# Marcus-Forte/moptimizer_0

Measured on NVIDIA B200. Metric: point2point_linearized_residuals_per_sec, higher is better.
Workload: dtype f32

## Files before the change

### moptimizer_0_b200/csrc/mopt_capi.cu

```cuda
#include <dlfcn.h>

#include <cmath>
#include <atomic>
#include <chrono>
#include <cstdlib>
#include <cstring>
#include <mutex>

#include "mopt_internal.h"

using namespace mopt;

namespace {
thread_local std::string g_last_error;
}
namespace mopt {
void set_last_error(const std::string& msg) { g_last_error = msg; }
int store_upload_async(mopt_store* st, int group, const void* host, int host_dtype, int64_t host_stride, int64_t first,
                       int64_t count);
}

namespace {
struct NcclApi {
  typedef struct ncclComm* comm_t;
// ... 167 lines not shown
  }
  return MOPT_OK;
}

void fill_cost(const mopt_problem* p, CostDev* c) {
  std::memset(c, 0, sizeof(*c));
  c->model = p->model; c->variant = p->variant; c->P = p->num_parameters; c->O = p->num_outputs;
  c->jacobian = p->jacobian; c->loss = p->loss; c->has_cov = p->has_covariance ? 1 : 0;
  c->compute_dtype = p->compute_dtype; c->loss_param = p->loss_param;
  c->manifold = p->manifold;
  c->rot_offset = (p->model == MOPT_MODEL_POINT2POINT || p->model == MOPT_MODEL_PINHOLE ||
                   p->model == MOPT_MODEL_PINHOLE_DISTORT) ? 3 : -1;
  if (p->model >= MOPT_MODEL_USER_BASE) c->rot_offset = user_model_rot_offset(p->model);
  c->so3_guard = ((p->flags & MOPT_FLAG_REFERENCE_FLOAT_GUARD) && p->compute_dtype == MOPT_F32) ? kSo3GuardF32 : kSo3GuardF64;
  const int O = p->num_outputs;
  for (int i = 0; i < O * O; ++i) c->cov[i] = p->has_covariance ? p->covariance[i] : ((i % (O + 1) == 0) ? 1.0 : 0.0);
  std::memcpy(c->consts, p->consts, sizeof(c->consts));
}

int stage_cost(mopt_ctx* ctx, int i, const mopt_problem* p) {
  CostDev c;
  fill_cost(p, &c);
  if (ctx->cached_valid[i] && std::memcmp(&c, &ctx->cached_cost[i], sizeof(c)) == 0) return MOPT_OK;
  MOPT_CUDA_TRY(cudaStreamSynchronize(ctx->stream));
  ctx->h_slot->cost = c;
  MOPT_CUDA_TRY(cudaMemcpyAsync(&ctx->d_slots[i].cost, &ctx->h_slot->cost, sizeof(CostDev), cudaMemcpyHostToDevice, ctx->stream));
  MOPT_CUDA_TRY(cudaStreamSynchronize(ctx->stream));
  ctx->cached_cost[i] = c;
  ctx->cached_valid[i] = true;
  return MOPT_OK;
}

PassArgs make_args(mopt_ctx* ctx, const mopt_store* st, int slot, int accumulate, int mode_override) {
  PassArgs a;
  std::memset(&a, 0, sizeof(a));
  for (int s = 0; s < kMaxStreams; ++s) a.streams.p[s] = st->streams[s];
  a.n = st->n;
  a.pb = &ctx->d_slots[slot].pb;
  a.cost = &ctx->d_slots[slot].cost;
  a.partials = ctx->d_partials;
  a.ticket = ctx->d_ticket;
  a.out = ctx->d_trial;
  a.accumulate = accumulate;
  a.mode_ptr = &ctx->d_lm->pass_mode;
  a.mode_override = mode_override;
  a.masked = st->may_have_invalid ? 1 : 0;
// ... 15 lines not shown
}

int launch_pass(mopt_ctx* ctx, const mopt_store* st, const mopt_problem* p, int slot, int accumulate, int mode_override,
                bool push, const XArg* fused_x = nullptr) {
  PassArgs a = make_args(ctx, st, slot, accumulate, mode_override);
  if (fused_x) {
    a.fused_setup = 1;
    a.x = *fused_x;
  }
  if (push && ctx->world > 1 && ctx->peers_open && ctx->exchange_enabled) {
    for (int r = 0; r < ctx->world; ++r) a.peer.base[r] = ctx->peer_base[r];
    a.peer.world = ctx->world;
    a.peer.rank = ctx->rank;
    a.peer.push = 1;
    a.peer.fused = ctx->fused_consumer ? 1 : 0;
    a.peer.err = ctx->d_xerr;
    a.peer.err_dev = ctx->d_xerr_dev;
    a.peer.seq = ++ctx->xseq;
  }
  PassLaunch L{ctx->stream, ctx->num_sms, ctx->ctas_per_sm, ctx->threads};
  L.affine_fd = (p->compute_dtype == MOPT_F32) ? !(p->flags & MOPT_FLAG_GENERIC_KERNEL)
                                               : ((p->flags & MOPT_FLAG_STABLE_FD) && !(p->flags & MOPT_FLAG_GENERIC_KERNEL));
  L.identity_cov = !p->has_covariance;
  if (p->model >= MOPT_MODEL_USER_BASE)
    return launch_user(L, ctx->device, p->model, p->jacobian != MOPT_JAC_ANALYTICAL, st->dtype, p->compute_dtype, a);
  if (p->model == MOPT_MODEL_POINT2POINT && p->jacobian == MOPT_JAC_ANALYTICAL)
    return launch_p2p_moment(L, st->dtype, p->compute_dtype, p->loss,
                             p->variant == MOPT_P2P_EXACT || p->variant == MOPT_P2P_LEFT, a);
  if (p->model == MOPT_MODEL_POINT2POINT && !(p->flags & MOPT_FLAG_GENERIC_KERNEL) &&
      !(st->dtype == MOPT_F64 && p->compute_dtype == MOPT_F32))
    return launch_p2p_moment(L, st->dtype, p->compute_dtype, p->loss, false, a);
  if (p->model == MOPT_MODEL_PINHOLE_DISTORT) return launch_wide(L, p->model, st->dtype, p->compute_dtype, a);
  return launch_dense(L, p->model, p->jacobian != MOPT_JAC_ANALYTICAL, st->dtype, p->compute_dtype, a);
}

int allreduce_trial(mopt_ctx* ctx, int P, int mode_override) {
  if (ctx->world <= 1 || !ctx->exchange_enabled) return MOPT_OK;
  if (ctx->peers_open) {
    if (ctx->fused_consumer) return MOPT_OK;
    peer_reduce_kernel<<<1, 64, 0, ctx->stream>>>(ctx->d_xbuf, ctx->world, ctx->xseq, ctx->d_trial, packed_size(P),
                                                  &ctx->d_lm->pass_mode, mode_override, ctx->d_xerr, ctx->d_xerr_dev);
    MOPT_CUDA_TRY(cudaGetLastError());
    return MOPT_OK;
  }
  if (!ctx->nccl_comm) {
    set_last_error("sharded context has neither a NCCL communicator nor an open peer exchange");
// ... 19 lines not shown

int check_exchange_alive(const mopt_ctx* ctx) {
  if (ctx->h_xerr && *reinterpret_cast<volatile int*>(ctx->h_xerr)) {
    set_last_error("an earlier peer exchange on this context timed out (a rank died); destroy the context");
    return MOPT_ERR_COMM;
  }
  return MOPT_OK;
}

int enqueue_pass(mopt_ctx* ctx, mopt_store* st, const mopt_problem* p, const double* x, int mode) {
  MOPT_TRY(check_exchange_alive(ctx));
  MOPT_CUDA_TRY(cudaSetDevice(ctx->device));
  MOPT_TRY(stage_cost(ctx, 0, p));
  const int P = p->num_parameters;
  XArg xa;
  std::memset(&xa, 0, sizeof(xa));
  if (P > 0) {
    MOPT_REQUIRE(x != nullptr, "null parameter vector");
    for (int i = 0; i < P; ++i) xa.v[i] = x[i];
  }
  if (can_fuse_setup(ctx, p, st)) {
    MOPT_TRY(launch_pass(ctx, st, p, 0, 0, mode, true, &xa));
  } else {
    setup_kernel<<<1, 32, 0, ctx->stream>>>(&ctx->d_slots[0], xa);
    MOPT_CUDA_TRY(cudaGetLastError());
    if (user_model_has_setup(p->model))
      MOPT_TRY(launch_user_setup(ctx->stream, ctx->device, p->model, &ctx->d_slots[0], nullptr, xa.v, P));
    MOPT_TRY(launch_pass(ctx, st, p, 0, 0, mode, true));
  }
  MOPT_TRY(allreduce_trial(ctx, P, mode));
  return MOPT_OK;
}

}

namespace mopt {
int setup_slot(mopt_ctx* ctx, int slot, const mopt_problem* problem, const double* x) {
  MOPT_TRY(stage_cost(ctx, slot, problem));
  XArg xa;
  std::memset(&xa, 0, sizeof(xa));
  for (int i = 0; i < problem->num_parameters; ++i) xa.v[i] = x[i];
  setup_kernel<<<1, 32, 0, ctx->stream>>>(&ctx->d_slots[slot], xa);
  MOPT_CUDA_TRY(cudaGetLastError());
  if (user_model_has_setup(problem->model))
    MOPT_TRY(launch_user_setup(ctx->stream, ctx->device, problem->model, &ctx->d_slots[slot], nullptr, xa.v,
                               problem->num_parameters));
  return MOPT_OK;
}
}

namespace {

int fetch_result(mopt_ctx* ctx, int P, double* H, double* b, double* sum) {
  MOPT_CUDA_TRY(cudaMemcpyAsync(ctx->h_result, ctx->d_trial, sizeof(double) * packed_size(P), cudaMemcpyDeviceToHost, ctx->stream));
  MOPT_CUDA_TRY(cudaStreamSynchronize(ctx->stream));
  if (ctx->h_xerr && *reinterpret_cast<volatile int*>(ctx->h_xerr)) {
    set_last_error("peer exchange timed out waiting for another rank");
    return MOPT_ERR_COMM;
  }
  unpack_result(*ctx->h_result, P, H, b, sum);
  return MOPT_OK;
}

int finish_lm(mopt_ctx* ctx, int P, double* x, mopt_lm_report* report, bool on_host = false) {
  LmState* hs = ctx->h_lm;
  constexpr int kFirstTrials = 48;
  const size_t first = offsetof(LmState, trials) + sizeof(mopt_lm_trial) * kFirstTrials;
  if (!on_host) {
    MOPT_CUDA_TRY(cudaMemcpyAsync(hs, ctx->d_lm, first, cudaMemcpyDeviceToHost, ctx->stream));
    MOPT_CUDA_TRY(cudaStreamSynchronize(ctx->stream));
  }
  if (!on_host && hs->num_trials > kFirstTrials) {
    const int more = (hs->num_trials < MOPT_MAX_TRACE ? hs->num_trials : MOPT_MAX_TRACE) - kFirstTrials;
    MOPT_CUDA_TRY(cudaMemcpyAsync(reinterpret_cast<char*>(hs) + first, reinterpret_cast<const char*>(ctx->d_lm) + first,
                                  sizeof(mopt_lm_trial) * size_t(more), cudaMemcpyDeviceToHost, ctx->stream));
    MOPT_CUDA_TRY(cudaStreamSynchronize(ctx->stream));
// ... 277 lines not shown

void mopt_lm_default_options(mopt_lm_options* o) {
  if (!o) return;
  o->max_iterations = 15;
  o->lm_max_iterations = 3;
  o->lambda_factor = 1e-9;
  o->scalar_dtype = MOPT_F64;
  o->speculative = 1;
  o->flags = MOPT_LM_STAGNATION_STOP;
}

int mopt_lm_minimize(mopt_ctx* ctx, int n_costs, mopt_store* const* stores, const mopt_problem* problems,
                     const mopt_lm_options* options, double* x, mopt_lm_report* report) try {
  MOPT_REQUIRE(ctx && stores && problems && x && report, "null argument");
  if (n_costs <= 0) {
    set_last_error("No cost function added!");
    return MOPT_ERR_INVALID_ARGUMENT;
  }
  MOPT_REQUIRE(n_costs <= MOPT_MAX_COSTS, "too many cost terms");
  mopt_lm_options opt;
  if (options) opt = *options; else mopt_lm_default_options(&opt);
  MOPT_REQUIRE(opt.max_iterations >= 0, "Optimization::max_iterations cannot be less than 0.");
  MOPT_REQUIRE(opt.lm_max_iterations >= 0, "lm_max_iterations cannot be negative");
  const int P = problems[0].num_parameters;
  MOPT_REQUIRE(P > 0 && P <= kMaxP, "bad num_parameters");
  for (int c = 0; c < n_costs; ++c) {
    MOPT_REQUIRE(stores[c] && stores[c]->ctx == ctx, "store does not belong to this context");
    MOPT_TRY(validate_problem(stores[c], &problems[c], true));
    MOPT_REQUIRE(problems[c].num_parameters == P, "all cost terms must share the parameter vector");
    MOPT_REQUIRE(problems[c].manifold == problems[0].manifold, "all cost terms must use the same manifold");
  }
  MOPT_TRY(check_exchange_alive(ctx));
  MOPT_CUDA_TRY(cudaSetDevice(ctx->device));
  std::memset(report, 0, offsetof(mopt_lm_report, trials));
  if (opt.max_iterations == 0) {
    report->status = MOPT_MAXIMUM_ITERATIONS_REACHED;
    return MOPT_OK;
  }
  for (int c = 0; c < n_costs; ++c) MOPT_TRY(stage_cost(ctx, c, &problems[c]));

  LmInit in;
  std::memset(&in, 0, sizeof(in));
  in.P = P; in.n_costs = n_costs; in.max_it = opt.max_iterations; in.lm_max_it = opt.lm_max_iterations;
  in.speculative = opt.speculative ? 1 : 0; in.scalar_f32 = (opt.scalar_dtype == MOPT_F32) ? 1 : 0;
  bool has_update = false;
  for (int c = 0; c < n_costs; ++c) has_update = has_update || (stores[c]->index != nullptr);
// ... 224 lines not shown
```

### moptimizer_0_b200/csrc/mopt_icp.cu

```cuda
#include <cmath>
#include <cstring>
#include <vector>

#include "mopt_internal.h"

using namespace mopt;

struct mopt_nn_index {
  mopt_ctx* ctx = nullptr;
  int dtype = MOPT_F64;
  int64_t m = 0;
  double max_dist = 0.0, cell = 0.0;
  double origin[3] = {0, 0, 0};
  int dims[3] = {1, 1, 1};
  int64_t ncells = 1;
  void* d_pts = nullptr;
  int* d_orig = nullptr;
  unsigned int* d_start = nullptr;
  long long* d_matched = nullptr;
};

namespace {

struct GridDesc {
// ... 150 lines not shown
          }
        }
      }
    }
    if (best_pos != 0xffffffffu) {
      tx[i] = ST(px[best_pos]);
      ty[i] = ST(py[best_pos]);
      tz[i] = ST(pz[best_pos]);
      ++local;
    } else {
      const ST no_match = ST(__longlong_as_double(0x7ff8000000000000LL));
      tx[i] = no_match;
      ty[i] = no_match;
      tz[i] = no_match;
    }
  }
  for (int off = 16; off >= 1; off >>= 1) local += __shfl_xor_sync(0xffffffffu, local, off);
  if ((threadIdx.x & 31) == 0 && local) atomicAdd(reinterpret_cast<unsigned long long*>(matched), (unsigned long long)local);
}

template <typename T>
int build_index(mopt_nn_index* ix, const void* host, int host_dtype) {
  mopt_ctx* ctx = ix->ctx;
  const int64_t m = ix->m;
  const size_t esz = sizeof(T);
  T* d_aos = nullptr;
  MOPT_CUDA_TRY(cudaMalloc(&d_aos, esz * 3 * size_t(m > 0 ? m : 1)));
  if ((host_dtype == MOPT_F32) == (sizeof(T) == 4)) {
    MOPT_CUDA_TRY(cudaMemcpyAsync(d_aos, host, esz * 3 * size_t(m), cudaMemcpyHostToDevice, ctx->stream));
  } else {
    std::vector<T> tmp(size_t(m) * 3);
    if (host_dtype == MOPT_F32) { const float* h = static_cast<const float*>(host); for (size_t i = 0; i < tmp.size(); ++i) tmp[i] = T(h[i]); }
    else { const double* h = static_cast<const double*>(host); for (size_t i = 0; i < tmp.size(); ++i) tmp[i] = T(h[i]); }
    MOPT_CUDA_TRY(cudaMemcpyAsync(d_aos, tmp.data(), esz * 3 * size_t(m), cudaMemcpyHostToDevice, ctx->stream));
    MOPT_CUDA_TRY(cudaStreamSynchronize(ctx->stream));
  }
  const int bb_blocks = 296;
  double* d_part = nullptr;
  MOPT_CUDA_TRY(cudaMalloc(&d_part, sizeof(double) * 6 * bb_blocks));
  bbox_kernel<T><<<bb_blocks, 256, 0, ctx->stream>>>(d_aos, m, d_part);
  MOPT_CUDA_TRY(cudaGetLastError());
  std::vector<double> part(6 * bb_blocks);
  MOPT_CUDA_TRY(cudaMemcpyAsync(part.data(), d_part, sizeof(double) * part.size(), cudaMemcpyDeviceToHost, ctx->stream));
  MOPT_CUDA_TRY(cudaStreamSynchronize(ctx->stream));
  cudaFree(d_part);
  double lo[3] = {1e300, 1e300, 1e300}, hi[3] = {-1e300, -1e300, -1e300};
// ... 51 lines not shown
  MOPT_CUDA_TRY(cudaMalloc(&ix->d_matched, sizeof(long long)));
  return MOPT_OK;
}

template <typename ST, typename T>
void launch_reassoc(mopt_store* st, mopt_nn_index* ix, const ParamBlock* pb, const LmState* gate) {
  GridDesc g;
  for (int k = 0; k < 3; ++k) { g.origin[k] = ix->origin[k]; g.dims[k] = ix->dims[k]; }
  g.inv_cell = 1.0 / ix->cell;
  const T* pts = static_cast<const T*>(ix->d_pts);
  int blocks = int(std::min<int64_t>((st->n + 255) / 256, 148 * 32));
  if (blocks < 1) blocks = 1;
  reassociate_kernel<ST, T><<<blocks, 256, 0, st->ctx->stream>>>(
      static_cast<const ST*>(st->streams[0]), static_cast<const ST*>(st->streams[1]), static_cast<const ST*>(st->streams[2]),
      static_cast<ST*>(st->streams[3]), static_cast<ST*>(st->streams[4]), static_cast<ST*>(st->streams[5]), st->n, pb, g,
      ix->max_dist, pts, pts + ix->m, pts + 2 * ix->m, ix->d_orig, ix->d_start, ix->d_matched, gate);
}

}

namespace mopt {

int enqueue_reassociate(mopt_store* st, const ParamBlock* pb, const LmState* gate) {
  mopt_nn_index* ix = st->index;
  if (!ix) return MOPT_OK;
  MOPT_CUDA_TRY(cudaMemsetAsync(ix->d_matched, 0, sizeof(long long), st->ctx->stream));
  if (st->dtype == MOPT_F32 && ix->dtype == MOPT_F32) launch_reassoc<float, float>(st, ix, pb, gate);
  else if (st->dtype == MOPT_F32 && ix->dtype == MOPT_F64) launch_reassoc<float, double>(st, ix, pb, gate);
  else if (st->dtype == MOPT_F64 && ix->dtype == MOPT_F32) launch_reassoc<double, float>(st, ix, pb, gate);
  else launch_reassoc<double, double>(st, ix, pb, gate);
  MOPT_CUDA_TRY(cudaGetLastError());
  st->may_have_invalid = true;
  return MOPT_OK;
}

}

extern "C" {

int mopt_nn_index_create(mopt_ctx* ctx, const void* host_xyz, int host_dtype, int index_dtype, int64_t m,
                         double max_distance, mopt_nn_index** out) try {
  MOPT_REQUIRE(ctx && out && (host_xyz || m == 0), "null argument");
  MOPT_REQUIRE(m >= 0 && m < (int64_t(1) << 31), "target cloud size must be below 2^31");
  MOPT_REQUIRE(max_distance > 0.0 && std::isfinite(max_distance), "max_distance must be positive");
  MOPT_REQUIRE((host_dtype == MOPT_F32 || host_dtype == MOPT_F64) && (index_dtype == MOPT_F32 || index_dtype == MOPT_F64),
               "bad dtype");
// ... 56 lines not shown
```

### moptimizer_0_b200/csrc/mopt_internal.h

```cpp
#pragma once

#include <cuda_runtime.h>

#include "mopt_common.cuh"
#include "mopt_lm.cuh"
#include "mopt_lm_mono.cuh"
#include "mopt_models.cuh"
#include "mopt_pass.cuh"

struct mopt_ctx {
  int device = 0;
  int num_sms = 148;
  cudaStream_t stream = nullptr;
  cudaStream_t copy_stream = nullptr;
  double* d_partials = nullptr;
  unsigned int* d_ticket = nullptr;
  mopt::PassResult* d_trial = nullptr;
  mopt::CostSlot* d_slots = nullptr;
  mopt::LmState* d_lm = nullptr;
  mopt::PassResult* h_result = nullptr;
  mopt::LmState* h_lm = nullptr;
  mopt::LmState* d_lm_host = nullptr;
  mopt::CostSlot* h_slot = nullptr;
  int* h_flags = nullptr;
// ... 1 lines not shown
  int flags_capacity = 0;
  mopt::CostDev cached_cost[MOPT_MAX_COSTS];
  bool cached_valid[MOPT_MAX_COSTS] = {false};
  void* d_stage[2] = {nullptr, nullptr};
  size_t stage_bytes = 0;
  cudaEvent_t ev_copy[2] = {nullptr, nullptr};
  cudaEvent_t ev_free[2] = {nullptr, nullptr};
  cudaEvent_t ev_batch[2] = {nullptr, nullptr};
  int ctas_per_sm = 0;
  int threads = 0;
  void* nccl_comm = nullptr;
  int rank = 0, world = 1;
  mopt::XSlot* d_xbuf = nullptr;
  mopt::XSlot* peer_base[mopt::kMaxWorld] = {nullptr};
  bool peers_open = false;
  bool exchange_enabled = true;
  bool fused_consumer = true;
  unsigned long long xseq = 0;
  int* h_xerr = nullptr;
  int* d_xerr = nullptr;
  unsigned long long* d_gen = nullptr;
  unsigned long long mono_gen = 0;
  int* d_xerr_dev = nullptr;
};

struct mopt_store {
  mopt_ctx* ctx = nullptr;
  int model = 0;
  int dtype = 0;
  int64_t n = 0;
  int nstreams = 0;
  void* streams[mopt::kMaxStreams] = {nullptr};
  struct mopt_nn_index* index = nullptr;
  bool may_have_invalid = false;
};

namespace mopt {

struct PassLaunch {
  cudaStream_t stream;
  int num_sms;
  int ctas_per_sm;
  int threads;
  bool affine_fd = true;
  bool identity_cov = false;
};

int launch_p2p_moment(const PassLaunch& L, int store_dtype, int compute_dtype, int loss, bool qrot, const PassArgs& a);
int launch_p2p_moment_gen2(const PassLaunch& L, int loss, bool qrot, const PassArgs& a);
int launch_p2p_lm_mono(const PassLaunch& L, int store_dtype, int compute_dtype, int loss, bool qrot, const PassArgs& a,
                       const MonoArgs& m);
int launch_dense(const PassLaunch& L, int model, bool numeric, int store_dtype, int compute_dtype, const PassArgs& a);

int setup_slot(mopt_ctx* ctx, int slot, const mopt_problem* problem, const double* x);
int enqueue_reassociate(mopt_store* st, const ParamBlock* pb, const LmState* gate);

int launch_wide(const PassLaunch& L, int model, int store_dtype, int compute_dtype, const PassArgs& a);

int launch_user(const PassLaunch& L, int device, int model, bool numeric, int store_dtype, int compute_dtype,
                const PassArgs& a);
int launch_user_setup(cudaStream_t stream, int device, int model, CostSlot* slot, const double* x_dev,
                      const double* x_host, int P);
int user_model_rot_offset(int model);
bool user_model_has_setup(int model);

int pick_grid(const void* kernel, int threads, const PassLaunch& L, int64_t work_items);

}
// ... 1 lines not shown
```

### moptimizer_0_b200/csrc/mopt_pass.cuh

```cuda
#pragma once

#include "mopt_common.cuh"
#include "mopt_setup.cuh"

namespace mopt {

constexpr int kMaxWorld = 8;
struct XSlot {
  double v[kPackedMax];
  unsigned long long seq;
  unsigned long long pad;
};
struct PeerArgs {
  XSlot* base[kMaxWorld];
  int world, rank, push;
  int fused;
  unsigned long long seq;
  int* err;
  int* err_dev;
};

struct PassArgs {
  PeerArgs peer;
  StreamPtrs streams;
  int64_t n;
  const ParamBlock* pb;
  const CostDev* cost;
  double* partials;
  unsigned int* ticket;
  PassResult* out;
  int accumulate;
  const int* mode_ptr;
  int mode_override;
  int masked;
  int fused_setup;
  int no_ring;
  XArg x;
};

#ifdef __CUDACC__

template <int NRAW, int THREADS>
__device__ __forceinline__ void grid_final_reduce(const double* partials, int G, double* s_tot) {
  constexpr int NW = THREADS / 32;
  const int lane = threadIdx.x & 31, warp = threadIdx.x >> 5;
  constexpr int ROWS = (NRAW + NW - 1) / NW;
  constexpr int RB = ROWS < 4 ? ROWS : 4;
  for (int q0 = 0; q0 < ROWS; q0 += RB) {
    double s[RB];
#pragma unroll
    for (int q = 0; q < RB; ++q) s[q] = 0.0;
    for (int c = lane; c < G; c += 32) {
      double v[RB];
#pragma unroll
      for (int q = 0; q < RB; ++q) {
        const int i = warp + (q0 + q) * NW;
        v[q] = (i < NRAW) ? __ldcg(partials + size_t(i) * G + c) : 0.0;
      }
#pragma unroll
// ... 1089 lines not shown
```

### moptimizer_0_b200/csrc/mopt_pass_p2p2.cu

```cuda
#include "mopt_internal.h"
#include "mopt_pass_p2p2.cuh"

namespace mopt {
namespace {

struct ShapeGen2 {
  static constexpr int THREADS = 384, STAGES = 2, U = 2, FLUSH = 16;
};

template <int LOSS, bool QROT, bool MASKED, bool FUSED, class S>
int launch_gen2_one(const PassLaunch& L, const PassArgs& a0) {
  auto kern = p2p_moment2_kernel<LOSS, QROT, MASKED, FUSED, S::THREADS, 1, S::STAGES, S::U, S::FLUSH, 0>;
  constexpr size_t smem = p2p2_ring_bytes(S::THREADS, S::STAGES, S::U);
  static bool configured[64] = {false};
  int dev = 0;
  MOPT_CUDA_TRY(cudaGetDevice(&dev));
  if (dev < 0 || dev >= 64 || !configured[dev]) {
    MOPT_CUDA_TRY(cudaFuncSetAttribute(kern, cudaFuncAttributeMaxDynamicSharedMemorySize, int(smem)));
    if (dev >= 0 && dev < 64) configured[dev] = true;
  }
  PassArgs a = a0;
  for (int k = 0; k < 6; ++k)
    if (reinterpret_cast<uintptr_t>(a.streams.p[k]) & 15u) a.no_ring = 1;
  const int64_t groups = a.n / 4;
  int64_t grid = int64_t(L.ctas_per_sm > 0 ? L.ctas_per_sm : 1) * L.num_sms;
  if (grid > L.num_sms) grid = L.num_sms;
  const int64_t need = (groups + S::THREADS - 1) / S::THREADS;
  if (need < grid) grid = need;
  if (grid < 1) grid = 1;
  kern<<<int(grid), S::THREADS, smem, L.stream>>>(a);
  MOPT_CUDA_TRY(cudaGetLastError());
  return MOPT_OK;
}

template <int LOSS, bool QROT, class S>
int launch_gen2_flags(const PassLaunch& L, const PassArgs& a) {
  if (a.masked)
    return a.fused_setup ? launch_gen2_one<LOSS, QROT, true, true, S>(L, a) : launch_gen2_one<LOSS, QROT, true, false, S>(L, a);
  return a.fused_setup ? launch_gen2_one<LOSS, QROT, false, true, S>(L, a) : launch_gen2_one<LOSS, QROT, false, false, S>(L, a);
}

template <class S>
int launch_gen2(const PassLaunch& L, int loss, bool qrot, const PassArgs& a) {
  switch (loss) {
    case MOPT_LOSS_NONE:
      return qrot ? launch_gen2_flags<MOPT_LOSS_NONE, true, S>(L, a) : launch_gen2_flags<MOPT_LOSS_NONE, false, S>(L, a);
    case MOPT_LOSS_GEMAN_MCCLURE:
      return qrot ? launch_gen2_flags<MOPT_LOSS_GEMAN_MCCLURE, true, S>(L, a)
                  : launch_gen2_flags<MOPT_LOSS_GEMAN_MCCLURE, false, S>(L, a);
    case MOPT_LOSS_HUBER:
      return qrot ? launch_gen2_flags<MOPT_LOSS_HUBER, true, S>(L, a) : launch_gen2_flags<MOPT_LOSS_HUBER, false, S>(L, a);
    default:
      set_last_error("unknown loss kind");
// ... 12 lines not shown
```

### moptimizer_0_b200/csrc/mopt_pass_p2p2.cuh

```cuda
#pragma once

#include "mopt_pass.cuh"

namespace mopt {
#ifdef __CUDACC__

__device__ __forceinline__ float2 bc2(float a) { return make_float2(a, a); }
__device__ __forceinline__ float2 neg2(float2 a) { return make_float2(-a.x, -a.y); }
__device__ __forceinline__ float2 fma2(float2 a, float2 b, float2 c) { return __ffma2_rn(a, b, c); }
__device__ __forceinline__ float2 add2(float2 a, float2 b) { return __fadd2_rn(a, b); }
__device__ __forceinline__ float2 sub2(float2 a, float2 b) { return __fadd2_rn(a, neg2(b)); }
__device__ __forceinline__ float2 mul2(float2 a, float2 b) { return __fmul2_rn(a, b); }

__device__ __forceinline__ unsigned smem_u32(const void* p) { return static_cast<unsigned>(__cvta_generic_to_shared(p)); }
__device__ __forceinline__ void mbar_init(uint64_t* bar, unsigned count) {
  asm volatile("mbarrier.init.shared::cta.b64 [%0], %1;" ::"r"(smem_u32(bar)), "r"(count) : "memory");
}
__device__ __forceinline__ void mbar_expect_tx(uint64_t* bar, unsigned bytes) {
  asm volatile("mbarrier.arrive.expect_tx.shared::cta.b64 _, [%0], %1;" ::"r"(smem_u32(bar)), "r"(bytes) : "memory");
}
__device__ __forceinline__ void mbar_arrive(uint64_t* bar) {
  asm volatile("mbarrier.arrive.shared::cta.b64 _, [%0];" ::"r"(smem_u32(bar)) : "memory");
}
__device__ __forceinline__ void mbar_wait(uint64_t* bar, unsigned parity) {
  asm volatile(
      "{\n"
      ".reg .pred p;\n"
      "MOPT_WAIT:\n"
      "mbarrier.try_wait.parity.shared::cta.b64 p, [%0], %1;\n"
      "@p bra MOPT_DONE;\n"
      "bra MOPT_WAIT;\n"
      "MOPT_DONE:\n"
      "}\n" ::"r"(smem_u32(bar)),
      "r"(parity)
      : "memory");
}
__device__ __forceinline__ void bulk_g2s(void* dst, const void* src, unsigned bytes, uint64_t* bar) {
  asm volatile("cp.async.bulk.shared::cluster.global.mbarrier::complete_tx::bytes [%0], [%1], %2, [%3];" ::"r"(smem_u32(dst)),
               "l"(src), "r"(bytes), "r"(smem_u32(bar))
               : "memory");
}

template <int LOSS>
__device__ __forceinline__ float loss_weight_fast(float k, float e2) {
  if constexpr (LOSS == MOPT_LOSS_HUBER) {
    float rs;
    asm("rsqrt.approx.ftz.f32 %0, %1;" : "=f"(rs) : "f"(fmaxf(e2, 1.17549435e-38f)));
    return (e2 <= k * k) ? 1.0f : k * rs;
  } else {
    return loss_weight<float>(LOSS, k, e2);
  }
}

template <int LOSS, bool QROT, bool MASKED>
__device__ __forceinline__ void p2p_moments_x2(const float (&R)[9], const float (&t)[3], float lossp, float2 px, float2 py,
                                               float2 pz, float2 yx, float2 yy, float2 yz, float2 (&acc)[kP2PRaw]) {
  bool skip0 = false, skip1 = false;
  if constexpr (MASKED) {
    skip0 = yx.x != yx.x; skip1 = yx.y != yx.y;
    if (skip0) { px.x = py.x = pz.x = 0.f; yx.x = t[0]; yy.x = t[1]; yz.x = t[2]; }
    if (skip1) { px.y = py.y = pz.y = 0.f; yx.y = t[0]; yy.y = t[1]; yz.y = t[2]; }
  }
  const float2 q0 = fma2(px, bc2(R[0]), fma2(py, bc2(R[1]), mul2(pz, bc2(R[2]))));
  const float2 q1 = fma2(px, bc2(R[3]), fma2(py, bc2(R[4]), mul2(pz, bc2(R[5]))));
// ... 21 lines not shown
  acc[19] = fma2(w2, r0, acc[19]); acc[20] = fma2(w2, r1, acc[20]); acc[21] = fma2(w2, r2, acc[21]);
  acc[22] = add2(acc[22], e2);
}

template <bool MASKED>
__device__ __forceinline__ void p2p_cost_x2(const float (&R)[9], const float (&t)[3], float2 px, float2 py, float2 pz,
                                            float2 yx, float2 yy, float2 yz, float2 (&acc)[kP2PRaw]) {
  const float2 r0 = sub2(add2(fma2(px, bc2(R[0]), fma2(py, bc2(R[1]), mul2(pz, bc2(R[2])))), bc2(t[0])), yx);
  const float2 r1 = sub2(add2(fma2(px, bc2(R[3]), fma2(py, bc2(R[4]), mul2(pz, bc2(R[5])))), bc2(t[1])), yy);
  const float2 r2 = sub2(add2(fma2(px, bc2(R[6]), fma2(py, bc2(R[7]), mul2(pz, bc2(R[8])))), bc2(t[2])), yz);
  float2 e2 = fma2(r0, r0, fma2(r1, r1, mul2(r2, r2)));
  if constexpr (MASKED) {
    if (yx.x != yx.x) e2.x = 0.f;
    if (yx.y != yx.y) e2.y = 0.f;
  }
  acc[22] = add2(acc[22], e2);
}

constexpr size_t p2p2_ring_bytes(int threads, int stages, int u) { return size_t(stages) * 6 * size_t(u) * threads * 16; }

template <int LOSS, bool QROT, bool MASKED, bool FUSED, int THREADS, int MINB, int STAGES, int U, int FLUSH_ROUNDS,
          int PF = 0>
__global__ void __launch_bounds__(THREADS, MINB) p2p_moment2_kernel(const PassArgs a) {
  const int mode = a.mode_override >= 0 ? a.mode_override : *a.mode_ptr;
  if (mode == PASS_SKIP) return;
  if (peer_failed(a)) return;
  constexpr int NW = THREADS / 32;
  constexpr int CHUNK = THREADS * U;

  __shared__ double s_warp[NW * 32];
  __shared__ double s_tot[32];
  __shared__ double s_set0[FUSED ? 12 : 1];
  __shared__ __align__(8) uint64_t s_full[STAGES > 0 ? STAGES : 1];
  __shared__ __align__(8) uint64_t s_empty[STAGES > 0 ? STAGES : 1];
  extern __shared__ __align__(128) unsigned char p2p2_ring[];
  float4* ring = reinterpret_cast<float4*>(p2p2_ring);

  const int lane = threadIdx.x & 31;
  const double* set0 = FUSED ? s_set0 : a.pb->sets[0];
  if constexpr (FUSED) {
    if (threadIdx.x == 0) {
      double xl[6];
#pragma unroll
      for (int i = 0; i < 6; ++i) xl[i] = a.x.v[i];
      p2p_fused_set0(a.cost, xl, s_set0);
    }
  }
  if constexpr (STAGES > 0) {
    if (threadIdx.x == 0) {
#pragma unroll
      for (int s = 0; s < STAGES; ++s) {
        mbar_init(&s_full[s], 1);
        mbar_init(&s_empty[s], NW);
      }
      asm volatile("fence.mbarrier_init.release.cluster;" ::: "memory");
    }
  }
  if constexpr (FUSED || STAGES > 0) __syncthreads();

  const float* __restrict__ sp[6];
#pragma unroll
  for (int k = 0; k < 6; ++k) sp[k] = static_cast<const float*>(a.streams.p[k]);

  const int64_t ngroups = a.n / 4;
  const int64_t stride = int64_t(gridDim.x) * CHUNK;
  const int64_t full_rounds = (STAGES > 0 && a.no_ring) ? 0 : ngroups / stride;

  auto issue_to = [&](int64_t rr, int s) {
    const int64_t g = rr * stride + int64_t(blockIdx.x) * CHUNK;
    mbar_expect_tx(&s_full[s], 6u * CHUNK * 16u);
#pragma unroll
    for (int k = 0; k < 6; ++k)
      bulk_g2s(ring + (size_t(s) * 6 + k) * CHUNK, reinterpret_cast<const float4*>(sp[k]) + g, CHUNK * 16u, &s_full[s]);
  };
  if constexpr (STAGES > 0) {
    if (threadIdx.x == 0)
      for (int rr = 0; rr < STAGES && rr < full_rounds; ++rr) issue_to(rr, rr);
  }
  auto prefetch_round = [&](int64_t rr) {
    if (PF > 0 && threadIdx.x == 0 && rr < full_rounds) {
      const int64_t g = rr * stride + int64_t(blockIdx.x) * CHUNK;
#pragma unroll
      for (int k = 0; k < 6; ++k) l2_prefetch_bulk(reinterpret_cast<const float4*>(sp[k]) + g, CHUNK * 16u);
    }
  };
  if constexpr (STAGES == 0 && PF > 0)
    for (int64_t rr = 0; rr < PF; ++rr) prefetch_round(rr);

  float R[9], t[3];
#pragma unroll
  for (int i = 0; i < 9; ++i) R[i] = float(set0[i]);
#pragma unroll
  for (int i = 0; i < 3; ++i) t[i] = float(set0[9 + i]);
  const float lossp = float(a.cost->loss_param);

  float2 acc[kP2PRaw];
#pragma unroll
  for (int i = 0; i < kP2PRaw; ++i) acc[i] = make_float2(0.f, 0.f);
  double dacc[1] = {0.0};

  auto flush = [&]() {
// ... 27 lines not shown
    float4 v[6];
#pragma unroll
    for (int k = 0; k < 6; ++k) v[k] = ld_stream(reinterpret_cast<const float4*>(sp[k]) + g);
    consume(v);
  };

  int since_flush = 0;
  if constexpr (STAGES > 0) {
    int s = 0;
    unsigned ph = 0;
    const float4* st = ring + threadIdx.x;
    for (int64_t r = 0; r < full_rounds; ++r) {
      mbar_wait(&s_full[s], ph);
      float4 v[U][6];
#pragma unroll
      for (int u = 0; u < U; ++u)
#pragma unroll
        for (int k = 0; k < 6; ++k) v[u][k] = st[(s * 6 + k) * CHUNK + u * THREADS];
      __syncwarp();
      if (lane == 0) mbar_arrive(&s_empty[s]);
      if (threadIdx.x == 0 && r + STAGES < full_rounds) {
        mbar_wait(&s_empty[s], ph);
        issue_to(r + STAGES, s);
      }
#pragma unroll
      for (int u = 0; u < U; ++u) consume(v[u]);
      if (++since_flush >= FLUSH_ROUNDS) {
        flush();
        since_flush = 0;
      }
      if (++s == STAGES) {
        s = 0;
        ph ^= 1u;
      }
    }
  } else {
    for (int64_t r = 0; r < full_rounds; ++r) {
      if (PF > 0) prefetch_round(r + PF);
      const int64_t g = r * stride + int64_t(blockIdx.x) * CHUNK + threadIdx.x;
      float4 v[U][6];
#pragma unroll
      for (int u = 0; u < U; ++u)
#pragma unroll
        for (int k = 0; k < 6; ++k) v[u][k] = ld_stream(reinterpret_cast<const float4*>(sp[k]) + g + u * THREADS);
#pragma unroll
      for (int u = 0; u < U; ++u) consume(v[u]);
// ... 7 lines not shown
    for (int64_t g = full_rounds * stride + int64_t(blockIdx.x) * THREADS + threadIdx.x; g < ngroups;
         g += int64_t(gridDim.x) * THREADS) {
      direct_group(g);
      if (++since_flush >= FLUSH_ROUNDS) {
        flush();
        since_flush = 0;
      }
    }
    if (blockIdx.x == 0 && threadIdx.x == 0) {
      for (int64_t i = ngroups * 4; i < a.n; ++i) {
        float2 one[kP2PRaw];
#pragma unroll
        for (int k = 0; k < kP2PRaw; ++k) one[k] = make_float2(0.f, 0.f);
        const float2 px = make_float2(sp[0][i], 0.f), py = make_float2(sp[1][i], 0.f), pz = make_float2(sp[2][i], 0.f);
        const float2 yx = make_float2(sp[3][i], t[0]), yy = make_float2(sp[4][i], t[1]), yz = make_float2(sp[5][i], t[2]);
        if (mode == PASS_COST) p2p_cost_x2<MASKED>(R, t, px, py, pz, yx, yy, yz, one);
        else p2p_moments_x2<LOSS, QROT, MASKED>(R, t, lossp, px, py, pz, yx, yy, yz, one);
#pragma unroll
        for (int k = 0; k < kP2PRaw; ++k) acc[k].x += one[k].x;
      }
    }
  }
  flush();
  p2p_finish<FUSED, THREADS>(a, mode, dacc, s_tot, s_warp);
}

#endif
}
```

### moptimizer_0_b200/csrc/mopt_peaks.cu

```cuda
#include <algorithm>
#include <chrono>
#include <cstring>
#include <vector>

#include "mopt_internal.h"

namespace {

using namespace mopt;

template <int ILP>
__global__ void __launch_bounds__(512) fma_peak_kernel(const float* bc, float* out, int iters) {
  const float b = bc[0], c = bc[1];
  float a[ILP];
#pragma unroll
  for (int k = 0; k < ILP; ++k) a[k] = float(threadIdx.x + k) * 1e-3f;
  for (int i = 0; i < iters; ++i) {
#pragma unroll
    for (int k = 0; k < ILP; ++k) a[k] = fmaf(a[k], b, c);
  }
  float s = 0.f;
#pragma unroll
  for (int k = 0; k < ILP; ++k) s += a[k];
  if (s == 123.456f) out[0] = s;
// ... 43 lines not shown
  for (int r = 0; r < reps; ++r) {
    MOPT_CUDA_TRY(cudaEventRecord(e0, stream));
    launch();
    MOPT_CUDA_TRY(cudaEventRecord(e1, stream));
    MOPT_CUDA_TRY(cudaEventSynchronize(e1));
    float ms = 0.f;
    MOPT_CUDA_TRY(cudaEventElapsedTime(&ms, e0, e1));
    best = std::min(best, ms);
  }
  cudaEventDestroy(e0);
  cudaEventDestroy(e1);
  MOPT_CUDA_TRY(cudaGetLastError());
  *best_ms = best;
  return MOPT_OK;
}

}

extern "C" int mopt_measure_peaks(mopt_ctx* ctx, mopt_peaks* out) try {
  MOPT_REQUIRE(ctx && out, "null argument");
  MOPT_CUDA_TRY(cudaSetDevice(ctx->device));
  std::memset(out, 0, sizeof(*out));
  cudaStream_t s = ctx->stream;
  float *d_bc = nullptr, *d_out = nullptr;
  MOPT_CUDA_TRY(cudaMalloc(&d_bc, 2 * sizeof(float)));
  MOPT_CUDA_TRY(cudaMalloc(&d_out, sizeof(float)));
  const float bc[2] = {0.999f, 1e-3f};
  MOPT_CUDA_TRY(cudaMemcpy(d_bc, bc, sizeof(bc), cudaMemcpyHostToDevice));
  constexpr int ILP = 8, THREADS = 512;
  const int grid = ctx->num_sms * 4;
  const int iters = 20000;
  const double thread_ops = double(grid) * THREADS * double(iters) * ILP;
  float ms = 0.f;
  MOPT_TRY(time_best(s, [&] { fma_peak_kernel<ILP><<<grid, THREADS, 0, s>>>(d_bc, d_out, iters); }, 5, &ms));
  out->fp32_fma_tflops = 2.0 * thread_ops / (ms * 1e-3) / 1e12;
  MOPT_TRY(time_best(s, [&] { fma2_peak_kernel<ILP><<<grid, THREADS, 0, s>>>(d_bc, d_out, iters); }, 5, &ms));
  out->fp32_fma2_tflops = 4.0 * thread_ops / (ms * 1e-3) / 1e12;
  out->issue_gwarp_inst_per_s = out->fp32_fma_tflops * 1e12 / 64.0 / 1e9;
  {
    const int64_t bytes = int64_t(2) << 30;
    float4* buf = nullptr;
    MOPT_CUDA_TRY(cudaMalloc(&buf, size_t(bytes)));
    MOPT_CUDA_TRY(cudaMemsetAsync(buf, 0, size_t(bytes), s));
    const int64_t n4 = bytes / 16;
    MOPT_TRY(time_best(s, [&] { read_peak_kernel<<<ctx->num_sms * 8, 256, 0, s>>>(buf, n4, d_out); }, 10, &ms));
    out->hbm_read_gbs = double(bytes) / (ms * 1e-3) / 1e9;
    cudaFree(buf);
  }
  cudaFree(d_bc);
  cudaFree(d_out);
  return MOPT_OK;
}
MOPT_ABI_CATCH

extern "C" int mopt_measure_h2d(mopt_ctx* ctx, uint64_t bytes, double seconds, double* gbs) try {
  MOPT_REQUIRE(ctx && gbs && bytes >= (1u << 20), "bad argument");
  MOPT_CUDA_TRY(cudaSetDevice(ctx->device));
  const size_t chunk = size_t(64) << 20;
  void *h = nullptr, *d = nullptr;
  MOPT_CUDA_TRY(cudaHostAlloc(&h, bytes, cudaHostAllocDefault));
  std::memset(h, 1, bytes);
  if (cudaMalloc(&d, bytes) != cudaSuccess) {
    cudaFreeHost(h);
    (void)cudaGetLastError();
    mopt::set_last_error("mopt_measure_h2d: out of device memory");
    return MOPT_ERR_OUT_OF_MEMORY;
  }
  cudaStream_t s = ctx->stream;
  auto sweep = [&] {
    for (size_t o = 0; o < bytes; o += chunk)
      cudaMemcpyAsync(static_cast<char*>(d) + o, static_cast<char*>(h) + o, std::min(chunk, size_t(bytes) - o),
                      cudaMemcpyHostToDevice, s);
  };
  sweep();
  MOPT_CUDA_TRY(cudaStreamSynchronize(s));
  const auto t0 = std::chrono::steady_clock::now();
  double elapsed = 0.0;
  uint64_t moved = 0;
  do {
    sweep();
    MOPT_CUDA_TRY(cudaStreamSynchronize(s));
    moved += bytes;
    elapsed = std::chrono::duration<double>(std::chrono::steady_clock::now() - t0).count();
  } while (elapsed < seconds);
  *gbs = double(moved) / elapsed / 1e9;
  cudaFree(d);
  cudaFreeHost(h);
  return MOPT_OK;
}
MOPT_ABI_CATCH
```

### moptimizer_0_b200/csrc/mopt_store.cu

```cuda
#include <cstring>

#include "mopt_internal.h"

using namespace mopt;

namespace {

template <typename HT, typename ST>
__global__ void deinterleave_kernel(const HT* __restrict__ aos, int64_t stride, int ncomp, ST* __restrict__ s0,
                                    ST* __restrict__ s1, ST* __restrict__ s2, int64_t first, int64_t count) {
  for (int64_t i = int64_t(blockIdx.x) * blockDim.x + threadIdx.x; i < count; i += int64_t(gridDim.x) * blockDim.x) {
    const HT* e = aos + i * stride;
    s0[first + i] = ST(e[0]);
    if (ncomp > 1) s1[first + i] = ST(e[1]);
    if (ncomp > 2) s2[first + i] = ST(e[2]);
  }
}

template <typename HT, typename ST>
__global__ void interleave_kernel(HT* __restrict__ aos, int ncomp, const ST* __restrict__ s0, const ST* __restrict__ s1,
                                  const ST* __restrict__ s2, int64_t first, int64_t count) {
  for (int64_t i = int64_t(blockIdx.x) * blockDim.x + threadIdx.x; i < count; i += int64_t(gridDim.x) * blockDim.x) {
    HT* e = aos + i * ncomp;
    e[0] = HT(s0[first + i]);
// ... 141 lines not shown

namespace mopt {

int store_upload_async(mopt_store* st, int group, const void* host, int host_dtype, int64_t host_stride, int64_t first,
                       int64_t count) {
  mopt_ctx* ctx = st->ctx;
  const ModelShape sh = model_shape(st->model);
  MOPT_REQUIRE(group == 0 || group == 1, "group must be 0 (A) or 1 (B)");
  const int ncomp = group == 0 ? sh.ncomp_a : sh.ncomp_b;
  MOPT_REQUIRE(ncomp > 0, "this model has no such data group");
  MOPT_REQUIRE(first >= 0 && count >= 0 && first + count <= st->n, "upload range outside the store");
  MOPT_REQUIRE(host_dtype == MOPT_F32 || host_dtype == MOPT_F64, "bad host dtype");
  if (count == 0) return MOPT_OK;
  MOPT_REQUIRE(host != nullptr, "null host pointer");
  if (host_stride == 0) host_stride = ncomp;
  MOPT_REQUIRE(host_stride >= ncomp, "host stride smaller than the component count");
  void* const* streams = st->streams + (group == 0 ? 0 : sh.NA);
  const size_t hsz = dtype_size(host_dtype);
  const size_t chunk_bytes_target = size_t(64) << 20;
  int64_t chunk_elems = int64_t(chunk_bytes_target / (hsz * size_t(host_stride)));
  if (chunk_elems < 1) chunk_elems = 1;
  if (chunk_elems > count) chunk_elems = count;
  MOPT_TRY(ensure_stage(ctx, size_t(chunk_elems) * size_t(host_stride) * hsz));
  int buf = 0;
  for (int64_t off = 0; off < count; off += chunk_elems, buf ^= 1) {
    const int64_t m = (count - off < chunk_elems) ? (count - off) : chunk_elems;
    const size_t bytes = (size_t(m - 1) * size_t(host_stride) + size_t(ncomp)) * hsz;
    MOPT_CUDA_TRY(cudaStreamWaitEvent(ctx->copy_stream, ctx->ev_free[buf], 0));
    MOPT_CUDA_TRY(cudaMemcpyAsync(ctx->d_stage[buf], static_cast<const char*>(host) + size_t(off) * size_t(host_stride) * hsz,
                                  bytes, cudaMemcpyHostToDevice, ctx->copy_stream));
    MOPT_CUDA_TRY(cudaEventRecord(ctx->ev_copy[buf], ctx->copy_stream));
    MOPT_CUDA_TRY(cudaStreamWaitEvent(ctx->stream, ctx->ev_copy[buf], 0));
    if (host_dtype == MOPT_F32 && st->dtype == MOPT_F32)
      launch_deinterleave<float, float>(ctx->stream, ctx->d_stage[buf], host_stride, ncomp, streams, first + off, m);
    else if (host_dtype == MOPT_F64 && st->dtype == MOPT_F32)
      launch_deinterleave<double, float>(ctx->stream, ctx->d_stage[buf], host_stride, ncomp, streams, first + off, m);
    else if (host_dtype == MOPT_F32 && st->dtype == MOPT_F64)
      launch_deinterleave<float, double>(ctx->stream, ctx->d_stage[buf], host_stride, ncomp, streams, first + off, m);
    else
      launch_deinterleave<double, double>(ctx->stream, ctx->d_stage[buf], host_stride, ncomp, streams, first + off, m);
    MOPT_CUDA_TRY(cudaGetLastError());
    MOPT_CUDA_TRY(cudaEventRecord(ctx->ev_free[buf], ctx->stream));
  }
  return MOPT_OK;
}

// ... 52 lines not shown
  MOPT_CUDA_TRY(cudaSetDevice(st->ctx->device));
  MOPT_TRY(store_upload_async(st, group, host, host_dtype, host_stride, first, count));
  MOPT_CUDA_TRY(cudaStreamSynchronize(st->ctx->stream));
  return MOPT_OK;
}
MOPT_ABI_CATCH

int mopt_store_download(mopt_store* st, int group, void* host, int host_dtype, int64_t first, int64_t count) try {
  MOPT_REQUIRE(st && host, "null store/host");
  mopt_ctx* ctx = st->ctx;
  MOPT_CUDA_TRY(cudaSetDevice(ctx->device));
  const ModelShape sh = model_shape(st->model);
  MOPT_REQUIRE(group == 0 || group == 1, "group must be 0 (A) or 1 (B)");
  const int ncomp = group == 0 ? sh.ncomp_a : sh.ncomp_b;
  MOPT_REQUIRE(ncomp > 0, "this model has no such data group");
  MOPT_REQUIRE(first >= 0 && count >= 0 && first + count <= st->n, "download range outside the store");
  MOPT_REQUIRE(host_dtype == MOPT_F32 || host_dtype == MOPT_F64, "bad host dtype");
  void* const* streams = st->streams + (group == 0 ? 0 : sh.NA);
  const size_t hsz = dtype_size(host_dtype);
  const int64_t chunk_elems_max = int64_t((size_t(64) << 20) / (hsz * ncomp));
  const int64_t chunk = count < chunk_elems_max ? count : chunk_elems_max;
  if (count == 0) return MOPT_OK;
  MOPT_TRY(ensure_stage(ctx, size_t(chunk) * ncomp * hsz));
  for (int64_t off = 0; off < count; off += chunk) {
    const int64_t m = (count - off < chunk) ? (count - off) : chunk;
    if (host_dtype == MOPT_F32 && st->dtype == MOPT_F32)
      launch_interleave<float, float>(ctx->stream, ctx->d_stage[0], ncomp, streams, first + off, m);
    else if (host_dtype == MOPT_F64 && st->dtype == MOPT_F32)
      launch_interleave<double, float>(ctx->stream, ctx->d_stage[0], ncomp, streams, first + off, m);
    else if (host_dtype == MOPT_F32 && st->dtype == MOPT_F64)
      launch_interleave<float, double>(ctx->stream, ctx->d_stage[0], ncomp, streams, first + off, m);
    else
      launch_interleave<double, double>(ctx->stream, ctx->d_stage[0], ncomp, streams, first + off, m);
    MOPT_CUDA_TRY(cudaGetLastError());
    MOPT_CUDA_TRY(cudaMemcpyAsync(static_cast<char*>(host) + size_t(off) * ncomp * hsz, ctx->d_stage[0],
                                  size_t(m) * ncomp * hsz, cudaMemcpyDeviceToHost, ctx->stream));
    MOPT_CUDA_TRY(cudaStreamSynchronize(ctx->stream));
  }
  return MOPT_OK;
}
MOPT_ABI_CATCH

int mopt_store_generate(mopt_store* st, const mopt_synth* desc) try {
  MOPT_REQUIRE(st && desc, "null store/desc");
  mopt_ctx* ctx = st->ctx;
  MOPT_CUDA_TRY(cudaSetDevice(ctx->device));
  SynthDev d;
  std::memset(&d, 0, sizeof(d));
  d.seed = desc->seed;
  d.first_index = desc->first_index;
  d.n_total = desc->n_total > 0 ? desc->n_total : st->n;
  for (int k = 0; k < 3; ++k) {
    d.lo[k] = float(desc->lo[k]);
    d.hi[k] = float(desc->hi[k]);
  }
  d.sigma = float(desc->noise_sigma);
  d.outlier_fraction = float(desc->outlier_fraction);
  d.outlier_range = float(desc->outlier_range);
  const int threads = 256;
  int64_t blocks = (st->n + threads - 1) / threads;
  if (blocks > 148 * 16) blocks = 148 * 16;
  if (blocks < 1) blocks = 1;
  const bool f32 = st->dtype == MOPT_F32;
  switch (st->model) {
    case MOPT_MODEL_POINT2POINT:
    case MOPT_MODEL_POINT_DIST: {
      double R[9];
      rodrigues_host(desc->gt + 3, R);
// ... 61 lines not shown
```

Baseline: 289.3.

## Add programmatic dependent launch and L2 evict-first hints to p2p moment pass

```diff
diff --git a/moptimizer_0_b200/csrc/mopt_capi.cu b/moptimizer_0_b200/csrc/mopt_capi.cu
--- a/moptimizer_0_b200/csrc/mopt_capi.cu
+++ b/moptimizer_0_b200/csrc/mopt_capi.cu
@@ -213,6 +213,7 @@
   CostDev c;
   fill_cost(p, &c);
   if (ctx->cached_valid[i] && std::memcmp(&c, &ctx->cached_cost[i], sizeof(c)) == 0) return MOPT_OK;
+  note_enqueue(ctx);
   MOPT_CUDA_TRY(cudaStreamSynchronize(ctx->stream));
   ctx->h_slot->cost = c;
   MOPT_CUDA_TRY(cudaMemcpyAsync(&ctx->d_slots[i].cost, &ctx->h_slot->cost, sizeof(CostDev), cudaMemcpyHostToDevice, ctx->stream));
@@ -274,6 +275,7 @@
   L.affine_fd = (p->compute_dtype == MOPT_F32) ? !(p->flags & MOPT_FLAG_GENERIC_KERNEL)
                                                : ((p->flags & MOPT_FLAG_STABLE_FD) && !(p->flags & MOPT_FLAG_GENERIC_KERNEL));
   L.identity_cov = !p->has_covariance;
+  L.pdl = ctx->pass_tail && ctx->world <= 1;
   if (p->model >= MOPT_MODEL_USER_BASE)
     return launch_user(L, ctx->device, p->model, p->jacobian != MOPT_JAC_ANALYTICAL, st->dtype, p->compute_dtype, a);
   if (p->model == MOPT_MODEL_POINT2POINT && p->jacobian == MOPT_JAC_ANALYTICAL)
@@ -339,13 +341,16 @@
   if (can_fuse_setup(ctx, p, st)) {
     MOPT_TRY(launch_pass(ctx, st, p, 0, 0, mode, true, &xa));
   } else {
+    note_enqueue(ctx);
     setup_kernel<<<1, 32, 0, ctx->stream>>>(&ctx->d_slots[0], xa);
     MOPT_CUDA_TRY(cudaGetLastError());
     if (user_model_has_setup(p->model))
       MOPT_TRY(launch_user_setup(ctx->stream, ctx->device, p->model, &ctx->d_slots[0], nullptr, xa.v, P));
     MOPT_TRY(launch_pass(ctx, st, p, 0, 0, mode, true));
   }
+  ctx->pass_tail = false;
   MOPT_TRY(allreduce_trial(ctx, P, mode));
+  ctx->pass_tail = ctx->world <= 1;
   return MOPT_OK;
 }
 
@@ -354,6 +359,7 @@
 namespace mopt {
 int setup_slot(mopt_ctx* ctx, int slot, const mopt_problem* problem, const double* x) {
   MOPT_TRY(stage_cost(ctx, slot, problem));
+  note_enqueue(ctx);
   XArg xa;
   std::memset(&xa, 0, sizeof(xa));
   for (int i = 0; i < problem->num_parameters; ++i) xa.v[i] = x[i];
@@ -369,6 +375,7 @@
 namespace {
 
 int fetch_result(mopt_ctx* ctx, int P, double* H, double* b, double* sum) {
+  note_enqueue(ctx);
   MOPT_CUDA_TRY(cudaMemcpyAsync(ctx->h_result, ctx->d_trial, sizeof(double) * packed_size(P), cudaMemcpyDeviceToHost, ctx->stream));
   MOPT_CUDA_TRY(cudaStreamSynchronize(ctx->stream));
   if (ctx->h_xerr && *reinterpret_cast<volatile int*>(ctx->h_xerr)) {
@@ -692,6 +699,7 @@
   if (options) opt = *options; else mopt_lm_default_options(&opt);
   MOPT_REQUIRE(opt.max_iterations >= 0, "Optimization::max_iterations cannot be less than 0.");
   MOPT_REQUIRE(opt.lm_max_iterations >= 0, "lm_max_iterations cannot be negative");
+  note_enqueue(ctx);
   const int P = problems[0].num_parameters;
   MOPT_REQUIRE(P > 0 && P <= kMaxP, "bad num_parameters");
   for (int c = 0; c < n_costs; ++c) {
diff --git a/moptimizer_0_b200/csrc/mopt_icp.cu b/moptimizer_0_b200/csrc/mopt_icp.cu
--- a/moptimizer_0_b200/csrc/mopt_icp.cu
+++ b/moptimizer_0_b200/csrc/mopt_icp.cu
@@ -196,6 +196,7 @@
 template <typename T>
 int build_index(mopt_nn_index* ix, const void* host, int host_dtype) {
   mopt_ctx* ctx = ix->ctx;
+  note_enqueue(ctx);
   const int64_t m = ix->m;
   const size_t esz = sizeof(T);
   T* d_aos = nullptr;
@@ -293,6 +294,7 @@
 namespace mopt {
 
 int enqueue_reassociate(mopt_store* st, const ParamBlock* pb, const LmState* gate) {
+  note_enqueue(st->ctx);
   mopt_nn_index* ix = st->index;
   if (!ix) return MOPT_OK;
   MOPT_CUDA_TRY(cudaMemsetAsync(ix->d_matched, 0, sizeof(long long), st->ctx->stream));
diff --git a/moptimizer_0_b200/csrc/mopt_internal.h b/moptimizer_0_b200/csrc/mopt_internal.h
--- a/moptimizer_0_b200/csrc/mopt_internal.h
+++ b/moptimizer_0_b200/csrc/mopt_internal.h
@@ -47,7 +47,10 @@
   unsigned long long* d_gen = nullptr;
   unsigned long long mono_gen = 0;
   int* d_xerr_dev = nullptr;
+  bool pass_tail = false;
 };
+
+inline void note_enqueue(mopt_ctx* ctx) { ctx->pass_tail = false; }
 
 struct mopt_store {
   mopt_ctx* ctx = nullptr;
@@ -69,6 +72,7 @@
   int threads;
   bool affine_fd = true;
   bool identity_cov = false;
+  bool pdl = false;
 };
 
 int launch_p2p_moment(const PassLaunch& L, int store_dtype, int compute_dtype, int loss, bool qrot, const PassArgs& a);
diff --git a/moptimizer_0_b200/csrc/mopt_pass.cuh b/moptimizer_0_b200/csrc/mopt_pass.cuh
--- a/moptimizer_0_b200/csrc/mopt_pass.cuh
+++ b/moptimizer_0_b200/csrc/mopt_pass.cuh
@@ -35,6 +35,7 @@
   int masked;
   int fused_setup;
   int no_ring;
+  int l2_keep_rounds;
   XArg x;
 };
 
diff --git a/moptimizer_0_b200/csrc/mopt_pass_p2p2.cu b/moptimizer_0_b200/csrc/mopt_pass_p2p2.cu
--- a/moptimizer_0_b200/csrc/mopt_pass_p2p2.cu
+++ b/moptimizer_0_b200/csrc/mopt_pass_p2p2.cu
@@ -1,5 +1,8 @@
 #include "mopt_internal.h"
 #include "mopt_pass_p2p2.cuh"
+
+#include <algorithm>
+#include <cstdlib>
 
 namespace mopt {
 namespace {
@@ -7,7 +10,12 @@
 struct ShapeGen2 {
   static constexpr int THREADS = 384, STAGES = 2, U = 2, FLUSH = 16;
 };
+constexpr int kP2PL2KeepMB = 64;
 
+int env_int(const char* name, int dflt) {
+  const char* e = getenv(name);
+  return (e && e[0]) ? atoi(e) : dflt;
+}
 template <int LOSS, bool QROT, bool MASKED, bool FUSED, class S>
 int launch_gen2_one(const PassLaunch& L, const PassArgs& a0) {
   auto kern = p2p_moment2_kernel<LOSS, QROT, MASKED, FUSED, S::THREADS, 1, S::STAGES, S::U, S::FLUSH, 0>;
@@ -28,7 +36,24 @@
   const int64_t need = (groups + S::THREADS - 1) / S::THREADS;
   if (need < grid) grid = need;
   if (grid < 1) grid = 1;
-  kern<<<int(grid), S::THREADS, smem, L.stream>>>(a);
+  const int64_t round_bytes = grid * S::THREADS * S::U * 16 * 6;
+  const int64_t keep = int64_t(env_int("MOPT_P2P_L2_KEEP_MB", kP2PL2KeepMB)) << 20;
+  a.l2_keep_rounds = keep > 0 ? int(std::min<int64_t>(keep / round_bytes, INT32_MAX)) : 0;
+  if (L.pdl && env_int("MOPT_P2P_PDL", 1) != 0) {
+    cudaLaunchAttribute attr[1];
+    attr[0].id = cudaLaunchAttributeProgrammaticStreamSerialization;
+    attr[0].val.programmaticStreamSerializationAllowed = 1;
+    cudaLaunchConfig_t cfg = {};
+    cfg.gridDim = dim3(unsigned(grid));
+    cfg.blockDim = dim3(S::THREADS);
+    cfg.dynamicSmemBytes = smem;
+    cfg.stream = L.stream;
+    cfg.attrs = attr;
+    cfg.numAttrs = 1;
+    MOPT_CUDA_TRY(cudaLaunchKernelEx(&cfg, kern, a));
+  } else {
+    kern<<<int(grid), S::THREADS, smem, L.stream>>>(a);
+  }
   MOPT_CUDA_TRY(cudaGetLastError());
   return MOPT_OK;
 }
diff --git a/moptimizer_0_b200/csrc/mopt_pass_p2p2.cuh b/moptimizer_0_b200/csrc/mopt_pass_p2p2.cuh
--- a/moptimizer_0_b200/csrc/mopt_pass_p2p2.cuh
+++ b/moptimizer_0_b200/csrc/mopt_pass_p2p2.cuh
@@ -40,6 +40,20 @@
                "l"(src), "r"(bytes), "r"(smem_u32(bar))
                : "memory");
 }
+__device__ __forceinline__ void bulk_g2s_hint(void* dst, const void* src, unsigned bytes, uint64_t* bar, uint64_t policy) {
+  asm volatile(
+      "cp.async.bulk.shared::cluster.global.mbarrier::complete_tx::bytes.L2::cache_hint [%0], [%1], %2, [%3], %4;" ::"r"(
+          smem_u32(dst)),
+      "l"(src), "r"(bytes), "r"(smem_u32(bar)), "l"(policy)
+      : "memory");
+}
+__device__ __forceinline__ uint64_t l2_policy_evict_first() {
+  uint64_t p;
+  asm volatile("createpolicy.fractional.L2::evict_first.b64 %0, 1.0;" : "=l"(p));
+  return p;
+}
+__device__ __forceinline__ void griddep_wait() { asm volatile("griddepcontrol.wait;" ::: "memory"); }
+__device__ __forceinline__ void griddep_launch_dependents() { asm volatile("griddepcontrol.launch_dependents;" ::: "memory"); }
 
 template <int LOSS>
 __device__ __forceinline__ float loss_weight_fast(float k, float e2) {
@@ -107,11 +121,10 @@
 template <int LOSS, bool QROT, bool MASKED, bool FUSED, int THREADS, int MINB, int STAGES, int U, int FLUSH_ROUNDS,
           int PF = 0>
 __global__ void __launch_bounds__(THREADS, MINB) p2p_moment2_kernel(const PassArgs a) {
-  const int mode = a.mode_override >= 0 ? a.mode_override : *a.mode_ptr;
-  if (mode == PASS_SKIP) return;
-  if (peer_failed(a)) return;
+  if (a.mode_override == PASS_SKIP) return;
   constexpr int NW = THREADS / 32;
   constexpr int CHUNK = THREADS * U;
+  static_assert(THREADS >= 64, "warp 0 feeds the ring while warp 1 runs the fused set-up");
 
   __shared__ double s_warp[NW * 32];
   __shared__ double s_tot[32];
@@ -122,15 +135,30 @@
   float4* ring = reinterpret_cast<float4*>(p2p2_ring);
 
   const int lane = threadIdx.x & 31;
-  const double* set0 = FUSED ? s_set0 : a.pb->sets[0];
-  if constexpr (FUSED) {
-    if (threadIdx.x == 0) {
-      double xl[6];
-#pragma unroll
-      for (int i = 0; i < 6; ++i) xl[i] = a.x.v[i];
-      p2p_fused_set0(a.cost, xl, s_set0);
-    }
-  }
+  const float* __restrict__ sp[6];
+#pragma unroll
+  for (int k = 0; k < 6; ++k) sp[k] = static_cast<const float*>(a.streams.p[k]);
+
+  const int64_t ngroups = a.n / 4;
+  const int64_t stride = int64_t(gridDim.x) * CHUNK;
+  const int64_t full_rounds = (STAGES > 0 && a.no_ring) ? 0 : ngroups / stride;
+
+  uint64_t pol_first = 0;
+  if (STAGES > 0 && threadIdx.x == 0 && a.l2_keep_rounds > 0) pol_first = l2_policy_evict_first();
+  auto issue_to = [&](int64_t rr, int s) {
+    const int64_t g = rr * stride + int64_t(blockIdx.x) * CHUNK;
+    mbar_expect_tx(&s_full[s], 6u * CHUNK * 16u);
+    if (a.l2_keep_rounds > 0 && rr >= a.l2_keep_rounds) {
+#pragma unroll
+      for (int k = 0; k < 6; ++k)
+        bulk_g2s_hint(ring + (size_t(s) * 6 + k) * CHUNK, reinterpret_cast<const float4*>(sp[k]) + g, CHUNK * 16u,
+                      &s_full[s], pol_first);
+    } else {
+#pragma unroll
+      for (int k = 0; k < 6; ++k)
+        bulk_g2s(ring + (size_t(s) * 6 + k) * CHUNK, reinterpret_cast<const float4*>(sp[k]) + g, CHUNK * 16u, &s_full[s]);
+    }
+  };
   if constexpr (STAGES > 0) {
     if (threadIdx.x == 0) {
 #pragma unroll
@@ -139,29 +167,31 @@
         mbar_init(&s_empty[s], NW);
       }
       asm volatile("fence.mbarrier_init.release.cluster;" ::: "memory");
+      for (int rr = 0; rr < STAGES && rr < full_rounds; ++rr) issue_to(rr, rr);
+      if (full_rounds <= STAGES) griddep_launch_dependents();
+    }
+  }
+  if constexpr (FUSED) {
+    if (threadIdx.x == 32) {
+      double xl[6];
+#pragma unroll
+      for (int i = 0; i < 6; ++i) xl[i] = a.x.v[i];
+      p2p_fused_set0(a.cost, xl, s_set0);
     }
   }
   if constexpr (FUSED || STAGES > 0) __syncthreads();
-
-  const float* __restrict__ sp[6];
-#pragma unroll
-  for (int k = 0; k < 6; ++k) sp[k] = static_cast<const float*>(a.streams.p[k]);
-
-  const int64_t ngroups = a.n / 4;
-  const int64_t stride = int64_t(gridDim.x) * CHUNK;
-  const int64_t full_rounds = (STAGES > 0 && a.no_ring) ? 0 : ngroups / stride;
-
-  auto issue_to = [&](int64_t rr, int s) {
-    const int64_t g = rr * stride + int64_t(blockIdx.x) * CHUNK;
-    mbar_expect_tx(&s_full[s], 6u * CHUNK * 16u);
-#pragma unroll
-    for (int k = 0; k < 6; ++k)
-      bulk_g2s(ring + (size_t(s) * 6 + k) * CHUNK, reinterpret_cast<const float4*>(sp[k]) + g, CHUNK * 16u, &s_full[s]);
-  };
-  if constexpr (STAGES > 0) {
-    if (threadIdx.x == 0)
-      for (int rr = 0; rr < STAGES && rr < full_rounds; ++rr) issue_to(rr, rr);
-  }
+  const bool late_wait = FUSED && a.mode_override >= 0 && !a.peer.push;
+  if (!late_wait) griddep_wait();
+
+  const int mode = a.mode_override >= 0 ? a.mode_override : *a.mode_ptr;
+  if (mode == PASS_SKIP || peer_failed(a)) {
+    if constexpr (STAGES > 0) {
+      if (threadIdx.x == 0)
+        for (int rr = 0; rr < STAGES && rr < full_rounds; ++rr) mbar_wait(&s_full[rr], 0);
+    }
+    return;
+  }
+  const double* set0 = FUSED ? s_set0 : a.pb->sets[0];
   auto prefetch_round = [&](int64_t rr) {
     if (PF > 0 && threadIdx.x == 0 && rr < full_rounds) {
       const int64_t g = rr * stride + int64_t(blockIdx.x) * CHUNK;
@@ -235,6 +265,7 @@
       if (threadIdx.x == 0 && r + STAGES < full_rounds) {
         mbar_wait(&s_empty[s], ph);
         issue_to(r + STAGES, s);
+        if (r + STAGES + 1 == full_rounds) griddep_launch_dependents();
       }
 #pragma unroll
       for (int u = 0; u < U; ++u) consume(v[u]);
@@ -288,6 +319,7 @@
     }
   }
   flush();
+  if (late_wait) griddep_wait();
   p2p_finish<FUSED, THREADS>(a, mode, dacc, s_tot, s_warp);
 }
 
diff --git a/moptimizer_0_b200/csrc/mopt_peaks.cu b/moptimizer_0_b200/csrc/mopt_peaks.cu
--- a/moptimizer_0_b200/csrc/mopt_peaks.cu
+++ b/moptimizer_0_b200/csrc/mopt_peaks.cu
@@ -89,6 +89,7 @@
   MOPT_CUDA_TRY(cudaSetDevice(ctx->device));
   std::memset(out, 0, sizeof(*out));
   cudaStream_t s = ctx->stream;
+  note_enqueue(ctx);
   float *d_bc = nullptr, *d_out = nullptr;
   MOPT_CUDA_TRY(cudaMalloc(&d_bc, 2 * sizeof(float)));
   MOPT_CUDA_TRY(cudaMalloc(&d_out, sizeof(float)));
@@ -134,6 +135,7 @@
     return MOPT_ERR_OUT_OF_MEMORY;
   }
   cudaStream_t s = ctx->stream;
+  note_enqueue(ctx);
   auto sweep = [&] {
     for (size_t o = 0; o < bytes; o += chunk)
       cudaMemcpyAsync(static_cast<char*>(d) + o, static_cast<char*>(h) + o, std::min(chunk, size_t(bytes) - o),
diff --git a/moptimizer_0_b200/csrc/mopt_store.cu b/moptimizer_0_b200/csrc/mopt_store.cu
--- a/moptimizer_0_b200/csrc/mopt_store.cu
+++ b/moptimizer_0_b200/csrc/mopt_store.cu
@@ -187,6 +187,7 @@
   if (chunk_elems < 1) chunk_elems = 1;
   if (chunk_elems > count) chunk_elems = count;
   MOPT_TRY(ensure_stage(ctx, size_t(chunk_elems) * size_t(host_stride) * hsz));
+  note_enqueue(ctx);
   int buf = 0;
   for (int64_t off = 0; off < count; off += chunk_elems, buf ^= 1) {
     const int64_t m = (count - off < chunk_elems) ? (count - off) : chunk_elems;
@@ -285,6 +286,7 @@
   const int64_t chunk = count < chunk_elems_max ? count : chunk_elems_max;
   if (count == 0) return MOPT_OK;
   MOPT_TRY(ensure_stage(ctx, size_t(chunk) * ncomp * hsz));
+  note_enqueue(ctx);
   for (int64_t off = 0; off < count; off += chunk) {
     const int64_t m = (count - off < chunk) ? (count - off) : chunk;
     if (host_dtype == MOPT_F32 && st->dtype == MOPT_F32)
@@ -307,6 +309,7 @@
 int mopt_store_generate(mopt_store* st, const mopt_synth* desc) try {
   MOPT_REQUIRE(st && desc, "null store/desc");
   mopt_ctx* ctx = st->ctx;
+  note_enqueue(ctx);
   MOPT_CUDA_TRY(cudaSetDevice(ctx->device));
   SynthDev d;
   std::memset(&d, 0, sizeof(d));
```

Result: faster. 294.6 (median of 6 runs) (+1.8%).
